# ModelTC/llmc

Hardware: AMD Instinct MI355X
Metric: layers/sec (GPTQ W4A16, Llama-3-8B Linear shapes, 128x2048 calib) (higher is better)
Workload: dtype bf16

## Files before the change

llmc_amd/_ffi.py:

```python
import ctypes as C
import os

import torch

_HERE = os.path.dirname(os.path.abspath(__file__))
LIB_PATH = os.path.join(_HERE, 'csrc', 'libllmc_hip.so')

F16, BF16, F32 = 0, 1, 2
F64 = 3
OUT_FAKE, OUT_I32, OUT_I8, OUT_U8 = 0, 1, 2, 3
SCALAR_QPARAM = 16
LINEAR_YBLOCKED = 4
FRACTIONAL_ZP = 32

_DT = {torch.float16: F16, torch.bfloat16: BF16, torch.float32: F32}

_i64, _i32, _f32, _f64, _vp, _sz = C.c_int64, C.c_int, C.c_float, C.c_double, C.c_void_p, C.c_size_t

SIGNATURES = {
    'llmc_hip_abi_version': (_i32, []),
    'llmc_hip_build_id': (C.c_char_p, []),
    'llmc_hip_last_error': (_i32, [C.c_char_p, _sz]),
    'llmc_hip_set_helper_streams': (_i32, [_i32]),
    'llmc_hip_set_cu_reserve': (_i32, [_i32]),
    'llmc_hip_set_option': (_i32, [C.c_char_p, _i32]),
    'llmc_hip_get_option': (_i32, [C.c_char_p]),
    'llmc_hip_option_name': (_i32, [_i32, C.c_char_p, _sz]),
    'llmc_minmax_qparams_ws_bytes': (_sz, [_i64, _i64]),
    'llmc_minmax_qparams': (_i32, [_vp, _i32, _i64, _i64, _i32, _i32, _f32, _f32, _vp, _vp, _vp, _vp]),
    'llmc_minmax_samples_max': (_i32, []),
    'llmc_minmax_samples_ws_bytes': (_sz, [_vp, _i32]),
    'llmc_minmax_samples': (_i32, [_vp, _vp, _i32, _i32, _vp, _vp, _vp, _vp]),
    'llmc_histc_ws_bytes': (_sz, [_i32]),
    'llmc_histc': (_i32, [_vp, _i32, _i64, _i32, _f32, _f32, _vp, _vp, _vp]),
    'llmc_mse_qparams': (_i32, [_vp, _i32, _i64, _i64, _i32, _i32, _f32, _f32, _i32, _i32, _f32, _vp, _vp, _vp, _vp, _vp]),
    'llmc_mse_qparams_panel': (_i32, [_vp, _i64, _i64, _i64, _i64, _i64, _i32, _i32, _f32, _f32, _i32, _i32, _f32, _vp,
                                      _vp, _i64, _i64, _vp]),
    'llmc_hqq_ws_bytes': (_sz, [_i64, _i64, _i32, _i64, _i32]),
    'llmc_hqq_optimize': (_i32, [_vp, _i32, _i64, _i64, _i64, _i32, _i64, _i32, _i32, _f32, _f32, _vp, _vp, _f32, _f32,
                                 _i32, _i32, _vp, _vp, _vp, _vp, _vp, _vp]),
    'llmc_quant_static': (_i32, [_vp, _i32, _i64, _i64, _vp, _i32, _vp, _i32, _f32, _f32, _i32, _vp, _vp]),
    'llmc_quant_dynamic_ws_bytes': (_sz, [_i64, _i64]),
    'llmc_quant_dynamic': (_i32, [_vp, _i32, _i64, _i64, _i32, _i32, _f32, _f32, _i32, _vp, _vp, _vp, _vp, _vp]),
    'llmc_pack_lsb': (_i32, [_vp, _i32, _i64, _i64, _i32, _vp, _vp]),
    'llmc_hessian_accum_ws_bytes': (_sz, [_i64, _i64, _i64]),
    'llmc_hessian_accum': (_i32, [_vp, _vp, _i32, _i64, _i64, _i64, _f64, _f64, _vp, _vp]),
    'llmc_hessian_accum_partials': (_i32, [_vp, _i32, _i64, _i64, _i64, _vp, _vp]),
    'llmc_hessian_accum_reduce': (_i32, [_vp, _i64, _i64, _i64, _f64, _f64, _vp, _vp]),
    'llmc_hessian_max_samples': (_i32, []),
    'llmc_hessian_accum_ptrs_ws_bytes': (_sz, [_vp, _i32, _i64, _i64]),
    'llmc_hessian_accum_ptrs': (_i32, [_vp, _vp, _vp, _i32, _i32, _i64, _i64, _f64, _f64, _vp, _vp]),
    'llmc_hessian_accum_ptrs_partials': (_i32, [_vp, _vp, _i32, _i32, _i64, _i64, _vp, _vp]),
    'llmc_hessian_accum_ptrs_reduce': (_i32, [_vp, _vp, _i32, _i64, _i64, _f64, _f64, _vp, _vp]),
    'llmc_hessian_accum_barrier_timeouts': (_i32, [_vp, _vp, _i32, _i64, _i64, _vp, _vp]),
    'llmc_hessian_max_problems': (_i32, []),
    'llmc_hessian_accum_multi_ws_bytes': (_sz, [_vp, _i32]),
    'llmc_hessian_accum_multi_partials': (_i32, [_vp, _i32, _i32, _vp, _vp]),
    'llmc_hessian_accum_multi_reduce': (_i32, [_vp, _i32, _vp, _vp]),
    'llmc_hessian_accum_multi_barrier_timeouts': (_i32, [_vp, _i32, _vp, _vp, _vp]),
    'llmc_gather_cols': (_i32, [_vp, _i64, _i64, _vp, _vp, _vp]),
    'llmc_hessian_prep_ws_bytes': (_sz, [_i64]),
    'llmc_hessian_prep': (_i32, [_vp, _vp, _i32, _i64, _i64, _vp, _f32, _vp, _vp, _vp, _vp]),
    'llmc_chol_inv_upper_ws_bytes': (_sz, [_i64]),
    'llmc_chol_inv_upper': (_i32, [_vp, _i64, _vp, _vp, _vp]),
    'llmc_hessian_prep_rev': (_i32, [_vp, _vp, _i32, _i64, _i64, _vp, _f32, _vp, _vp, _vp, _vp]),
    'llmc_chol_inv_upper_rev': (_i32, [_vp, _vp, _i64, _vp, _vp, _vp]),
    'llmc_gptq_quantize_ws_bytes': (_sz, [_i64, _i64]),
    'llmc_gptq_quantize': (_i32, [_vp, _vp, _i64, _i64, _i32, _f32, _f32, _i64, _i32, _vp, _vp, _vp, _vp, _vp,
                                  _i32, _vp, _vp]),
    'llmc_gptq_quantize_cols': (_i32, [_vp, _vp, _i64, _i64, _i64, _i32, _f32, _f32, _i64, _i32, _vp, _vp, _vp, _vp, _vp,
                                       _i32, _vp, _vp]),
    'llmc_gptq_quantize_fp8_cols': (_i32, [_vp, _vp, _i64, _i64, _i64, _i32, _i64, _i32, _vp, _vp, _vp, _vp, _i32, _vp, _vp]),
    'llmc_gptq_quantize_mse_ws_bytes': (_sz, [_i64, _i64]),
    'llmc_gptq_quantize_mse': (_i32, [_vp, _vp, _i64, _i64, _i64, _i32, _f32, _f32, _i64, _i32, _i32, _i32, _f32, _vp, _vp,
                                      _vp, _vp, _i32, _vp, _vp]),
    'llmc_spqr_quantize_ws_bytes': (_sz, [_i64, _i64]),
    'llmc_spqr_quantize': (_i32, [_vp, _vp, _i64, _i64, _f32, _f32, _i64, _f32, _i32, _f32, _f32, _f32, _f32, _vp, _vp,
                                  _vp, _vp, _vp, _i32, _vp, _vp]),
    'llmc_awq_act_mean_ws_bytes': (_sz, [_i64, _i64]),
    'llmc_awq_act_mean': (_i32, [_vp, _i32, _i64, _i64, _vp, _vp, _vp]),
    'llmc_awq_weight_mean_ws_bytes': (_sz, [_i64, _i64]),
    'llmc_awq_weight_mean': (_i32, [_vp, _i32, _i64, _i64, _i64, _vp, _vp, _vp]),
    'llmc_awq_scales': (_i32, [_vp, _vp, _i32, _i64, _f64, _i32, _vp, _vp]),
    'llmc_awq_scale_fakequant': (_i32, [_vp, _vp, _i32, _i64, _i64, _i64, _i32, _f32, _f32, _vp, _vp]),
    'llmc_div_cols': (_i32, [_vp, _vp, _i32, _i64, _i64, _vp, _vp]),
    'llmc_div_cols_kt': (_i32, [_vp, _vp, _i32, _i64, _i64, _vp, _vp]),
    'llmc_mul_cols': (_i32, [_vp, _vp, _i32, _i64, _i64, _vp]),
    'llmc_clamp_groups': (_i32, [_vp, _i32, _i64, _i64, _i64, _vp, _vp, _vp]),
    'llmc_linear_eval_ws_bytes': (_sz, [_i64, _i64, _i64]),
    'llmc_linear_eval': (_i32, [_vp, _vp, _i32, _i64, _i64, _i64, _i32, _vp, _vp, _vp, _vp, _vp]),
    'llmc_linear_eval_yblocked_bytes': (_sz, [_i64, _i64]),
    'llmc_ktile_pack': (_i32, [_vp, _i32, _i64, _i64, _vp, _vp]),
    'llmc_linear_eval_kt': (_i32, [_vp, _vp, _i32, _i64, _i64, _i64, _i32, _vp, _vp, _vp, _vp, _vp]),
    'llmc_awq_clip_search_ws_bytes': (_sz, [_i64, _i64, _i64, _i64]),
    'llmc_awq_clip_search': (_i32, [_vp, _vp, _i32, _i64, _i64, _i64, _i64, _i32, _i32, _i32, _i32, _f32, _f32,
                                    _vp, _vp, _vp, _vp]),
    'llmc_awq_clip_errs': (_i32, [_vp, _vp, _i32, _i64, _i64, _i64, _i64, _i32, _i32, _i32, _i32, _f32, _f32, _vp, _vp]),
    'llmc_awq_clip_errs_cand': (_i32, [_vp, _vp, _vp, _vp, _i32, _i64, _i64, _i64, _i64, _i64, _i32, _vp, _vp]),
    'llmc_fp8_quant_ws_bytes': (_sz, [_i64, _i64]),
    'llmc_fp8_quant': (_i32, [_vp, _i32, _i64, _i64, _i32, _vp, _vp, _i32, _i32, _vp, _vp]),
    'llmc_fpx_quant_ws_bytes': (_sz, [_i64, _i64]),
    'llmc_fpx_quant': (_i32, [_vp, _i32, _i64, _i64, _vp, _i64, _i32, _vp, _vp, _i32, _i32, _vp, _vp]),
    'llmc_fp4_pack': (_i32, [_vp, _i64, _i64, _vp, _vp]),
    'llmc_fpx_dequant': (_i32, [_vp, _i32, _i32, _vp, _i32, _i64, _i64, _vp, _i32, _vp]),
    'llmc_fp8_block_quant': (_i32, [_vp, _i32, _i64, _i64, _i32, _f32, _i32, _vp, _vp, _vp]),
    'llmc_fp8_block_dequant': (_i32, [_vp, _vp, _i64, _i64, _i32, _i32, _vp, _vp]),
    'llmc_fp8_act_quant': (_i32, [_vp, _i32, _i64, _i32, _vp, _vp, _vp]),
    'llmc_fp8_block_gemm': (_i32, [_vp, _vp, _vp, _vp, _i64, _i64, _i64, _i32, _vp, _vp, _vp]),
    'llmc_pack_awq_gemm': (_i32, [_vp, _i32, _vp, _i32, _vp, _i64, _i64, _i64, _vp, _vp, _vp, _vp]),
    'llmc_col_stats_ws_bytes': (_sz, [_i64, _i64]),
    'llmc_col_stats': (_i32, [_vp, _i32, _i64, _i64, _i32, _vp, _vp, _vp, _vp]),
    'llmc_smooth_scales': (_i32, [_vp, _vp, _i32, _i64, _f64, _f64, _vp, _vp]),
    'llmc_osplus_scale': (_i32, [_vp, _vp, _vp, _i64, _i32, _i64, _vp, _vp]),
    'llmc_osplus_act_step_tier': (_i32, [_i32, _i64]),
    'llmc_osplus_act_step': (_i32, [_vp, _vp, _i32, _i64, _i64, _i32, _i32, _f32, _f32, _i32, _vp, _vp]),
    'llmc_hadamard': (_i32, [_vp, _vp, _i32, _i64, _i64, _i64, _vp, _i32, _f64, _vp]),
    'llmc_test_sgemm': (_i32, [_vp, _vp, _vp, _i64, _i64, _i64, _i32, _i32, _i32, _i32, _i32, _i32, _i32, _i32,
                               _i32, _i32, _vp]),
    'llmc_test_sgemm_phased': (_i32, [_vp, _vp, _vp, _i64, _i64, _i64, _i32, _i32, _i32, _i32, _i32, _vp]),
    'llmc_test_gemm3': (_i32, [_vp, _vp, _vp, _i64, _i64, _i64, _i32, _i32, _i32, _i32, _i32, _i32, _i32, _i32, _vp]),
    'llmc_test_gemm3_planes': (_i32, [_vp, _vp, _vp, _i64, _i64, _i64, _i32, _i32, _i32, _i32, _i32, _vp, _vp]),
    'llmc_test_gemm3s_stamps': (_i32, [_vp]),
    'llmc_test_gptq_rider_plan': (_i32, [_i64, _i64, _i64, _i64, _i32, _vp, _i32]),
    'llmc_test_gptq_pipe_plan': (_i32, [_i64, _i64, _i64, _i64, _i32, _vp, _i32]),
    'llmc_test_chol_plan': (_i32, [_i64, _i32, _i32, _vp, _i32]),
    'llmc_test_gemm_route': (_i32, [_vp, _vp]),
}



class HessianProblem(C.Structure):
    _fields_ = [('H', _vp), ('dstate', _vp), ('X_list_host', _vp), ('T_list_host', _vp), ('n', _i32), ('K', _i64),
                ('ldx', _i64), ('n_before', _f64), ('n_after', _f64)]


_lib = None


class LlmcHipError(RuntimeError):
    pass


def lib():
    global _lib
    if _lib is None:
        if not os.path.exists(LIB_PATH):
            raise LlmcHipError(
                f'{LIB_PATH} not found: the HIP extension is required (run `python -m llmc_amd.build`). '
                'llmc_amd has no CPU fallback.')
        handle = C.CDLL(LIB_PATH)
        for name, (res, args) in SIGNATURES.items():
            fn = getattr(handle, name)
            fn.restype = res
            fn.argtypes = args
        ver = handle.llmc_hip_abi_version()
        if ver != 1:
            raise LlmcHipError(f'libllmc_hip.so ABI version {ver} != 1')
        if not os.environ.get('LLMC_SKIP_BUILD_ID_CHECK'):
            from . import build as _build
            have, want = handle.llmc_hip_build_id().decode(), _build.source_digest()
            if have != want:
                raise LlmcHipError(f'{LIB_PATH} is stale: built from sources {have}, csrc/ is {want} '
                                   '(run `python -m llmc_amd.build`; LLMC_SKIP_BUILD_ID_CHECK=1 skips this check)')
        _lib = handle
        _apply_startup_options()
    return _lib


HOST_OPTIONS = {
    'awq_kt': 1,
    'awq_y_bytes': (1 << 32) - (1 << 20),
    'k3_fused_prep': 1,
}

_HOST_DEFAULTS = dict(HOST_OPTIONS)


def reset_options():
    HOST_OPTIONS.update(_HOST_DEFAULTS)
    if _lib is not None:
        for k in library_options():
            _lib.llmc_hip_set_option(k.encode(), 0)


def set_option(key, value):
    if key in HOST_OPTIONS:
        prev, HOST_OPTIONS[key] = HOST_OPTIONS[key], int(value)
        return prev
    prev = lib().llmc_hip_set_option(key.encode(), int(value))
    if prev < 0:
        raise ValueError(f'unknown option {key!r} (library keys: {library_options()}; host keys: {sorted(HOST_OPTIONS)})')
    return prev


def get_option(key):
    if key in HOST_OPTIONS:
        return HOST_OPTIONS[key]
    v = lib().llmc_hip_get_option(key.encode())
    if v < 0:
        raise ValueError(f'unknown option {key!r}')
    return v


def library_options():
    out, buf, i = [], C.create_string_buffer(64), 0
    while lib().llmc_hip_option_name(i, buf, 64) > 0:
        out.append(buf.value.decode())
        i += 1
    return out


class option:

    def __init__(self, **kv):
        self.kv = kv

    def __enter__(self):
        self.prev = {k: set_option(k, v) for k, v in self.kv.items()}
        return self

    def __exit__(self, *exc):
        for k, v in self.prev.items():
            set_option(k, v)
        return False


def _apply_startup_options():
    spec = os.environ.get('LLMC_OPTIONS', '')
    for item in filter(None, (x.strip() for x in spec.split(','))):
        k, _, v = item.partition('=')
        set_option(k.strip(), int(v or 1))


def last_error():
    buf = C.create_string_buffer(512)
    lib().llmc_hip_last_error(buf, 512)
    return buf.value.decode(errors='replace')


def check(rc, what):
    if rc == 0:
        return
    msg = last_error()
    if rc == -22:
        raise ValueError(f'{what}: invalid argument: {msg}')
    if rc == -95:
        raise NotImplementedError(f'{what}: unsupported: {msg}')
    raise LlmcHipError(f'{what}: HIP error: {msg}')


def dt(t):
    try:
        return _DT[t.dtype if isinstance(t, torch.Tensor) else t]
    except KeyError:
        raise ValueError(f'unsupported dtype {t.dtype if isinstance(t, torch.Tensor) else t}')


def require_gpu(*tensors):
    cur = None
    for t in tensors:
        if t is None:
            continue
        if not t.is_cuda:
            raise LlmcHipError(
                'llmc_amd operators run on MI355X only (tensor is on '
                f'{t.device}); there is no CPU fallback. Use oracle/ for CPU checks in tests.')
        if cur is None:
            cur = torch.cuda.current_device()
        if t.device.index != cur:
            raise LlmcHipError(f'tensor lives on {t.device} but the current device is cuda:{cur}: wrap the call in '
                               '`with torch.cuda.device(tensor.device)` (hipSetDevice is the caller\'s job)')


def ptr(t):
    return 0 if t is None else t.data_ptr()


def stream():
    return torch.cuda.current_stream().cuda_stream


def workspace(nbytes, device):
    if nbytes <= 0:
        return None
    return torch.empty(int(nbytes), dtype=torch.uint8, device=device)


class helper_streams:

    def __init__(self, enable):
        self.enable = int(bool(enable))

    def __enter__(self):
        self.prev = lib().llmc_hip_set_helper_streams(self.enable)

    def __exit__(self, *exc):
        lib().llmc_hip_set_helper_streams(self.prev)
        return False


class cu_reserve:

    def __init__(self, n):
        self.n = int(n)

    def __enter__(self):
        self.prev = lib().llmc_hip_set_cu_reserve(self.n)

    def __exit__(self, *exc):
        lib().llmc_hip_set_cu_reserve(self.prev)
        return False
```

llmc_amd/csrc/abi.hip:

```cpp
#include <mutex>
#include <set>
#include <utility>
#include "common.h"

namespace llmc {
static thread_local char g_last_error[512] = "";
static thread_local int g_helper_streams = 1;
bool helper_streams_enabled() { return g_helper_streams != 0; }
static thread_local int g_cu_reserve = 0;
int cu_reserve() { return g_cu_reserve; }
static thread_local int g_opt[OPT_COUNT] = {};
int opt(int id) { return (id >= 0 && id < OPT_COUNT) ? g_opt[id] : 0; }
static const char* const g_opt_names[OPT_COUNT] = {
    "k3_fp32", "k3_no_gemm6", "k3_no_planes", "k3_split_far", "k4_split_far", "k4_err_rowmajor", "gptq_generic",
    "gemm3_nospec", "gemm3s_min_tiles", "no_shortk", "linear_nosplit", "fp8_exact_div", "side_cu_mask", "k1_batch_off", "k1_fp32_diag", "fp8_no_packed16", "gemm3s_no_dma", "sgemm_no_wide", "gemm3_no_wide", "no_riders"};

void set_last_error(const char* where, hipError_t e) {
    snprintf(g_last_error, sizeof(g_last_error), "%s: %s (%d)", where, hipGetErrorString(e), (int)e);
}
void set_last_error_msg(const char* msg) { snprintf(g_last_error, sizeof(g_last_error), "%s", msg); }

static std::mutex g_dev_mu;
static int g_cu_count[LLMC_MAX_DEVICES] = {};
static std::set<std::pair<int, const void*>> g_lds_attr_done;

int device_cu_count() {
    int dev = 0;
    if (hipGetDevice(&dev) != hipSuccess || dev < 0 || dev >= LLMC_MAX_DEVICES) return 256;
    std::lock_guard<std::mutex> lk(g_dev_mu);
    if (g_cu_count[dev] == 0) {
        int n = 0;
        if (hipDeviceGetAttribute(&n, hipDeviceAttributeMultiprocessorCount, dev) != hipSuccess || n <= 0) n = 256;
        g_cu_count[dev] = n;
    }
    return g_cu_count[dev];
}

int ensure_dynamic_lds(const void* fn, int bytes) {
    int dev = 0;
    LLMC_HIP_CHECK(hipGetDevice(&dev));
    std::lock_guard<std::mutex> lk(g_dev_mu);
    auto key = std::make_pair(dev, fn);
    if (g_lds_attr_done.count(key)) return LLMC_OK;
    LLMC_HIP_CHECK(hipFuncSetAttribute(fn, hipFuncAttributeMaxDynamicSharedMemorySize, bytes));
    g_lds_attr_done.insert(key);
    return LLMC_OK;
}
}

extern "C" int llmc_hip_set_helper_streams(int enable) {
    int prev = llmc::g_helper_streams;
    llmc::g_helper_streams = enable ? 1 : 0;
    return prev;
}

extern "C" int llmc_hip_set_option(const char* key, int value) {
    if (!key || value < 0) return LLMC_EINVAL;
    for (int i = 0; i < llmc::OPT_COUNT; ++i)
        if (strcmp(key, llmc::g_opt_names[i]) == 0) {
            const int prev = llmc::g_opt[i];
            llmc::g_opt[i] = value;
            return prev;
        }
    llmc::set_last_error_msg("llmc_hip_set_option: unknown key");
    return LLMC_EINVAL;
}

extern "C" int llmc_hip_get_option(const char* key) {
    if (!key) return LLMC_EINVAL;
    for (int i = 0; i < llmc::OPT_COUNT; ++i)
        if (strcmp(key, llmc::g_opt_names[i]) == 0) return llmc::g_opt[i];
    return LLMC_EINVAL;
}

extern "C" int llmc_hip_option_name(int index, char* buf_host, size_t n) {
    if (index < 0 || index >= llmc::OPT_COUNT || !buf_host || n == 0) return LLMC_EINVAL;
    strncpy(buf_host, llmc::g_opt_names[index], n - 1);
    buf_host[n - 1] = 0;
    return (int)strlen(buf_host);
}

extern "C" int llmc_hip_set_cu_reserve(int n_cus) {
    int prev = llmc::g_cu_reserve;
    llmc::g_cu_reserve = n_cus < 0 ? 0 : n_cus;
    return prev;
}

extern "C" int llmc_hip_abi_version(void) { return LLMC_HIP_ABI_VERSION; }

#ifndef LLMC_BUILD_ID
#define LLMC_BUILD_ID "unknown"
#endif
extern "C" const char* llmc_hip_build_id(void) { return LLMC_BUILD_ID; }

extern "C" int llmc_hip_last_error(char* buf_host, size_t n) {
    if (!buf_host || n == 0) return (int)strlen(llmc::g_last_error);
    strncpy(buf_host, llmc::g_last_error, n - 1);
    buf_host[n - 1] = 0;
    return (int)strlen(buf_host);
}
```

llmc_amd/csrc/common.h:

```cpp
#pragma once
#include <hip/hip_runtime.h>
#include <stdint.h>
#include <string.h>
#include <stdio.h>
#include <stdlib.h>

#include "../../include/llmc_hip.h"

namespace llmc {

void set_last_error(const char* where, hipError_t e);
void set_last_error_msg(const char* msg);

#define LLMC_HIP_CHECK(expr)                                   \
    do {                                                       \
        hipError_t _e = (expr);                                \
        if (_e != hipSuccess) {                                \
            ::llmc::set_last_error(#expr, _e);                 \
            return LLMC_EIO;                                   \
        }                                                      \
    } while (0)

#define LLMC_LAUNCH_CHECK()                                    \
    do {                                                       \
        hipError_t _e = hipGetLastError();                     \
        if (_e != hipSuccess) {                                \
            ::llmc::set_last_error("kernel launch", _e);       \
            return LLMC_EIO;                                   \
        }                                                      \
    } while (0)

#define LLMC_REQUIRE(cond, msg)                                \
    do {                                                       \
        if (!(cond)) {                                         \
            ::llmc::set_last_error_msg(msg);                   \
            return LLMC_EINVAL;                                \
        }                                                      \
    } while (0)

static constexpr int LLMC_MAX_DEVICES = 64;
int device_cu_count();
int ensure_dynamic_lds(const void* fn, int bytes);
int cu_reserve();
bool helper_streams_enabled();

enum Opt : int {
    OPT_K3_FP32 = 0,
    OPT_K3_NO_GEMM6,
    OPT_K3_NO_PLANES,
    OPT_K3_SPLIT_FAR,
    OPT_K4_SPLIT_FAR,
    OPT_K4_ERR_ROWMAJOR,
    OPT_GPTQ_GENERIC,
    OPT_GEMM3_NOSPEC,
    OPT_GEMM3S_MIN_TILES,
    OPT_NO_SHORTK,
    OPT_LINEAR_NOSPLIT,
    OPT_FP8_EXACT_DIV,
    OPT_SIDE_CU_MASK,
    OPT_K1_BATCH_OFF,
    OPT_K1_FP32_DIAG,
    OPT_FP8_NO_PACKED16,
    OPT_GEMM3S_NO_DMA,
    OPT_SGEMM_NO_WIDE,
    OPT_GEMM3_NO_WIDE,
    OPT_NO_RIDERS,
    OPT_COUNT
};
int opt(int id);
#ifdef LLMC_LAB
static inline const char* lab_env(const char* k) { return getenv(k); }
#endif

static inline int dtype_size(int dt) { return dt == LLMC_F32 ? 4 : 2; }
static inline bool dtype_ok(int dt) { return dt == LLMC_F16 || dt == LLMC_BF16 || dt == LLMC_F32; }

struct f16_t { uint16_t u; };
struct bf16_t { uint16_t u; };

template <typename T> struct dt_of;
template <> struct dt_of<f16_t> { static constexpr int value = LLMC_F16; };
template <> struct dt_of<bf16_t> { static constexpr int value = LLMC_BF16; };
template <> struct dt_of<float> { static constexpr int value = LLMC_F32; };

#define DISPATCH_DT(dt, ...)                                              \
    switch (dt) {                                                         \
        case LLMC_F16: { using T = ::llmc::f16_t; __VA_ARGS__; break; }   \
        case LLMC_BF16: { using T = ::llmc::bf16_t; __VA_ARGS__; break; } \
        default: { using T = float; __VA_ARGS__; break; }                 \
    }

__device__ __forceinline__ float f16_bits_to_f32(uint16_t u) {
    _Float16 h;
    __builtin_memcpy(&h, &u, 2);
    return (float)h;
}
__device__ __forceinline__ uint16_t f32_to_f16_bits(float v) {
    asm volatile("" : "+v"(v));
    _Float16 h = (_Float16)v;
    uint16_t u;
    __builtin_memcpy(&u, &h, 2);
    return u;
}
__device__ __forceinline__ float bf16_bits_to_f32(uint16_t u) {
    return __uint_as_float(((uint32_t)u) << 16);
}
__device__ __forceinline__ uint16_t f32_to_bf16_bits(float v) {
    const __bf16 h = (__bf16)v;
    uint16_t u;
    __builtin_memcpy(&u, &h, 2);
    return u;
}

__device__ __forceinline__ float opaque_f32(float v) {
    asm volatile("" : "+v"(v));
    return v;
}

__device__ __forceinline__ float rnd(float v, int dt) {
    if (dt == LLMC_F16) return f16_bits_to_f32(f32_to_f16_bits(v));
    if (dt == LLMC_BF16) return bf16_bits_to_f32(f32_to_bf16_bits(v));
    return v;
}
template <int DT> __device__ __forceinline__ float rndc(float v) {
    if constexpr (DT == LLMC_F16) return f16_bits_to_f32(f32_to_f16_bits(v));
    else if constexpr (DT == LLMC_BF16) return bf16_bits_to_f32(f32_to_bf16_bits(v));
    else return v;
}

__device__ __forceinline__ float load_as_f32(const void* p, int64_t i, int dt) {
    if (dt == LLMC_F16) return f16_bits_to_f32(((const uint16_t*)p)[i]);
    if (dt == LLMC_BF16) return bf16_bits_to_f32(((const uint16_t*)p)[i]);
    return ((const float*)p)[i];
}
__device__ __forceinline__ void store_from_f32(void* p, int64_t i, int dt, float v) {
    if (dt == LLMC_F16) ((uint16_t*)p)[i] = f32_to_f16_bits(v);
    else if (dt == LLMC_BF16) ((uint16_t*)p)[i] = f32_to_bf16_bits(v);
    else ((float*)p)[i] = v;
}

template <typename T> __device__ __forceinline__ float to_f32(T v);
template <> __device__ __forceinline__ float to_f32<f16_t>(f16_t v) { return f16_bits_to_f32(v.u); }
template <> __device__ __forceinline__ float to_f32<bf16_t>(bf16_t v) { return bf16_bits_to_f32(v.u); }
template <> __device__ __forceinline__ float to_f32<float>(float v) { return v; }

template <typename T> __device__ __forceinline__ T from_f32(float v);
template <> __device__ __forceinline__ f16_t from_f32<f16_t>(float v) { return f16_t{f32_to_f16_bits(v)}; }
template <> __device__ __forceinline__ bf16_t from_f32<bf16_t>(float v) { return bf16_t{f32_to_bf16_bits(v)}; }
template <> __device__ __forceinline__ float from_f32<float>(float v) { return v; }

__host__ __device__ __forceinline__ int promote(int a, int b) {
    if (a == b) return a;
    return LLMC_F32;
}

template <typename T> struct vec16 {
    static constexpr int N = 16 / sizeof(T);
    T v[N];
};

__device__ __forceinline__ float wave_max(float v, int width) {
    for (int o = width >> 1; o > 0; o >>= 1) v = fmaxf(v, __shfl_xor(v, o, 64));
    return v;
}
__device__ __forceinline__ float wave_min(float v, int width) {
    for (int o = width >> 1; o > 0; o >>= 1) v = fminf(v, __shfl_xor(v, o, 64));
    return v;
}
__device__ __forceinline__ float wave_sum(float v, int width) {
    for (int o = width >> 1; o > 0; o >>= 1) v += __shfl_xor(v, o, 64);
    return v;
}

static inline int64_t ceil_div64(int64_t a, int64_t b) { return (a + b - 1) / b; }
static inline int capped_grid(int64_t items, int64_t per_block, int64_t cap) {
    const int64_t b = ceil_div64(items, per_block);
    return (int)(b < 1 ? 1 : (b > cap ? cap : b));
}
static inline int pow2_ceil(int64_t x) {
    int p = 1;
    while (p < x) p <<= 1;
    return p;
}

}
```

llmc_amd/csrc/gptq_loop.hip:

```cpp
#include "gptq_block_kernels.h"
#include "pipe_lanes.h"

using namespace llmc;

static constexpr int GRP = 4;
static constexpr int GW = BS * GRP;

extern "C" size_t llmc_gptq_quantize_ws_bytes(int64_t R, int64_t K) {
    if (R <= 0 || K <= 0) return 0;
    return 3 * (size_t)((R + 3) & ~(int64_t)3) * GW * sizeof(float);
}

extern "C" int llmc_gptq_quantize(float* W, const float* Hinv, int64_t R, int64_t K, int sym, float qmin,
                                  float qmax, int64_t group_size, int static_groups, const int32_t* col_group,
                                  float* scales, float* zeros, float* Wout, float* losses, int blocksize,
                                  void* ws, llmc_stream_t stream) {
    return llmc_gptq_quantize_cols(W, Hinv, R, K, K, sym, qmin, qmax, group_size, static_groups, col_group, scales,
                                   zeros, Wout, losses, blocksize, ws, stream);
}

struct MseSearch { int round_zp, nsteps, grid; float norm; };

struct Piece { int64_t c0, c1; int k0, k1; Lane lane; };
static constexpr int CARRIERS = GRP;
static_assert(CARRIERS % RIDER_PASSES == 0 && GRP % RIDER_PASSES == 0, "a group's carrying launches and phases divide into the passes");

static int far_pieces(int64_t gend, int64_t K, bool merged, int rider_cols, Piece* p) {
    const int64_t gend2 = gend + GW < K ? gend + GW : K, gend3 = gend2 + GW < K ? gend2 + GW : K;
    if (!merged) {
        p[0] = Piece{gend, gend2, 0, GW, CHAIN}, p[1] = Piece{gend2, gend3, 0, GW, BULK}, p[2] = Piece{gend3, K, 0, GW, BULK};
        return 1 + (gend2 < K) + (gend3 < K);
    }
    const int64_t rw = (int64_t)rider_cols * 128, rspan = (CARRIERS / RIDER_PASSES) * rw;
    const int64_t p0 = (rider_cols > 0 && gend2 < K) ? (gend2 > K - rspan ? gend2 : K - rspan) : K;
    p[0] = Piece{gend, p0, 0, GW, CHAIN};
    int n = 1;
    const int kd = GW / RIDER_PASSES;
    for (int pass = 0; pass < RIDER_PASSES; ++pass)
        for (int64_t c = p0; c < K; c += rw) p[n++] = Piece{c, c + rw < K ? c + rw : K, pass * kd, (pass + 1) * kd, RIDE};
    return n;
}

struct ColCall {
    float* W; const float* U; float* Wout; float* losses; float* scales; float* zeros; const int32_t* col_group;
    int64_t R, K, NQ;
    bool ekm; int64_t Rp, err_ld; float* ErrBuf[3];
    int ng, gsz, static_mode, sym; float qmin, qmax;
    const MseSearch* mse;
    int kind;

    float* err(int group, int64_t k) const { return ErrBuf[group % 3] + (ekm ? k * Rp : k); }
    int64_t group_end(int64_t g0) const { return g0 + GW < NQ ? g0 + GW : NQ; }
    int64_t near_end(int64_t g0) const { return group_end(g0) == NQ ? K : group_end(g0); }
    int count(int64_t i1) const { return (int)(NQ - i1 < BS ? NQ - i1 : BS); }

    GptqBlockArgs block(int64_t i1) const {
        GptqBlockArgs a;
        a.W = W; a.U = U; a.Wout = Wout; a.losses = losses;
        a.Err = err((int)(i1 / GW), i1 % GW); a.err_ld = (int)err_ld; a.err_kmajor = ekm ? 1 : 0;
        a.scales = scales; a.zeros = zeros; a.col_group = mse ? nullptr : col_group; a.col_gsz = mse ? gsz : 1 << 30;
        a.R = R; a.K = (int)K; a.i1 = (int)i1; a.count = count(i1); a.ng = ng; a.gsz = static_mode ? BS : gsz;
        a.static_mode = static_mode; a.sym = sym; a.qmin = qmin; a.qmax = qmax;
        return a;
    }
    SgemmArgs product(const float* A, int64_t row0, int kd, int64_t c0, int64_t c1, int phase_len) const {
        SgemmArgs g{};
        g.A = A; g.lda = err_ld; g.B = U + row0 * K + c0; g.ldb = K; g.C = W + c0; g.ldc = K;
        g.M = g.M_last = (int)R; g.N = g.N_last = (int)(c1 - c0); g.Kd = g.Kd_last = kd;
        g.epilogue = SG_SUB; g.batch = 1; g.phase_len = phase_len;
        return g;
    }
    SgemmArgs near(int64_t i1) const {
        const int64_t g0 = i1 - i1 % GW, c0 = (i1 + count(i1)) & ~(int64_t)3;
        return product(err((int)(i1 / GW), i1 % GW), i1, count(i1), c0, near_end(g0), 0);
    }
    SgemmArgs far(int group, int64_t c0, int64_t c1, int k0, int k1) const {
        return product(err(group, k0), (int64_t)group * GW + k0, k1 - k0, c0, c1, BS);
    }
    RiderArgs riders(int group, const Piece& q, int nchain) const {
        RiderArgs ra{};
        wide::wide_operands<2>(far(group, q.c0, q.c1, q.k0, q.k1), ra.w);
        ra.nchain = nchain; ra.per = (nchain % 8 == 0 && ra.w.tm % 8 == 0) ? ra.w.tm / 8 : 0;
        return ra;
    }
};

enum { PLAN_BLOCK = 0, PLAN_NEAR = 1, PLAN_NEAR_FAR = 2, PLAN_FAR = 3, PLAN_FLUSH = 4, PLAN_W = 12 };
static const int32_t PLAN_BLANK[PLAN_W] = {0, 0, 0, 0, -1, -1, -1, 0, 0, -1, 0, 0};

struct Sink {
    const ColCall& o; const Lanes& ln; PlanRec* rec;
    void add(int lane, int kind, int group, int64_t w0, int64_t w1, int err_rd, int err_wr, int rgroup, int64_t r0, int64_t r1, int rerr,
             int k0, int k1) const {
        const int32_t v[PLAN_W] = {kind, group, (int32_t)w0, (int32_t)w1, err_rd, err_wr, rgroup, (int32_t)r0, (int32_t)r1, rerr, k0, k1};
        rec->row(v, lane);
    }
    int err_index(const float* pe) const { return (int)((size_t)(pe - o.ErrBuf[0]) / ((size_t)o.Rp * GW)); }
    void k_range(int group, const float* B, int64_t c0, int kd, int* k0, int* k1) const {
        *k0 = (int)((B - o.U - c0) / o.K - (int64_t)group * GW);
        *k1 = *k0 + kd;
        if (kd == GW) *k0 = *k1 = 0;
    }
    int product(int kind, int group, const SgemmArgs& g, hipStream_t st) const {
        if (!rec) return sgemm_launch(g, o.ekm, false, st);
        const int64_t c0 = g.C - o.W;
        int k0 = 0, k1 = 0;
        if (kind != PLAN_NEAR) k_range(group, g.B, c0, g.Kd, &k0, &k1);
        add(ln.lane_of(st), kind, group, c0, c0 + g.N, err_index(g.A), -1, -1, 0, 0, -1, k0, k1);
        return LLMC_OK;
    }
    int in_block(int group, const GptqBlockArgs& a, int variant, int nt, int grid, const RiderArgs* ra, int rgroup) const {
        const hipStream_t st = ln.s[CHAIN];
        if (rec) {
            int64_t r0 = 0, r1 = 0;
            int rerr = -1, k0 = 0, k1 = 0;
            if (ra) {
                r0 = ra->w.C - o.W, r1 = r0 + (int64_t)ra->w.tn * 128, rerr = err_index(ra->w.A);
                k_range(rgroup, ra->w.B, r0, ra->w.nst * wide::W_K, &k0, &k1);
            }
            add(CHAIN, PLAN_BLOCK, group, a.i1, a.i1 + a.count, -1, err_index(a.Err), rgroup, r0, r1, rerr, k0, k1);
            return LLMC_OK;
        }
        return o.kind == QK_E4M3 ? gptq_launch_in_block_e4m3(a, variant, nt, grid, ra, st)
             : o.kind == QK_E5M2 ? gptq_launch_in_block_e5m2(a, variant, nt, grid, ra, st)
                                 : launch_in_block<QK_INT>(a, variant, nt, grid, ra, st);
    }
};

static int rider_quota(const ColCall& o, bool merged, int nt, int grid) {
    if (!merged || opt(OPT_NO_RIDERS) || !o.ekm || nt != GBT || o.R % 128 || o.K % 128 || o.NQ <= GW || o.K <= 2 * (int64_t)GW) return 0;
    const int free_cus = device_cu_count() - grid;
    if (sgemm_route(o.far(0, 2 * GW, o.K, 0, GW), true, false).wide_form != 2 || free_cus <= 0 || 2 * grid < device_cu_count()) return 0;
    return (int)(free_cus / (o.R / 128));
}

static int gptq_cols_impl(float* W, const float* Hinv, int64_t R, int64_t K, int64_t n_quant, int sym, float qmin,
                          float qmax, int64_t group_size, int static_groups, const int32_t* col_group, float* scales,
                          float* zeros, float* Wout, float* losses, int blocksize, void* ws, llmc_stream_t stream,
                          const MseSearch* mse, PlanRec* rec = nullptr, int kind = QK_INT) {
    LLMC_REQUIRE(W && Hinv && Wout && scales && ws && R > 0 && K > 0, "gptq_quantize: null/empty argument");
    LLMC_REQUIRE(n_quant > 0 && n_quant <= K, "gptq_quantize: n_quant must be in (0, K]");
    LLMC_REQUIRE(blocksize == BS, "gptq_quantize: blocksize must be 128");
    LLMC_REQUIRE(K % 4 == 0 && K < (1 << 30), "gptq_quantize: K must be a multiple of 4");
    LLMC_REQUIRE(sym || zeros, "gptq_quantize: zeros required for asymmetric");
    const bool per_channel = group_size <= 0;
    const int static_mode = static_groups || per_channel || mse != nullptr;
    const int gsz = (int)group_size;
    if (!static_mode || mse) {
        if (!(gsz == 16 || gsz == 32 || gsz == 64 || gsz == 128)) {
            set_last_error_msg("gptq_quantize: dynamic group qparams need group_size in {16,32,64,128}");
            return LLMC_ENOTSUP;
        }
    } else if (!per_channel) {
        LLMC_REQUIRE(col_group != nullptr, "gptq_quantize: col_group required with static groups");
    }
    const bool ekm = !opt(OPT_K4_ERR_ROWMAJOR);
    const int64_t Rp = (R + 3) & ~(int64_t)3;
    const ColCall o{W, Hinv, Wout, losses, scales, zeros, per_channel ? nullptr : col_group, R, K, n_quant,
                    ekm, Rp, ekm ? Rp : GW, {(float*)ws, (float*)ws + (size_t)Rp * GW, (float*)ws + 2 * (size_t)Rp * GW},
                    per_channel ? 1 : (int)ceil_div64(K, group_size), gsz, static_mode, sym, qmin, qmax, mse, kind};
    Lanes ln((hipStream_t)stream, rec);
    const Sink sink{o, ln, rec};
    const bool merged = !ln.piped() && !opt(OPT_K4_SPLIT_FAR);
    const int nt = R >= 16384 ? 1024 : GBT;
    const int grid = (int)ceil_div64(R, nt / 16);
    const int rider_cols = rider_quota(o, merged, nt, grid);
    const bool force_generic = opt(OPT_GPTQ_GENERIC) != 0;
    Piece pc[1 + CARRIERS];
    int np = 0, next = 0, fg = 0;
    auto flush = [&]() -> int {
        for (; next < np; ++next)
            LLMC_TRY(sink.product(PLAN_FLUSH, fg, o.far(fg, pc[next].c0, pc[next].c1, pc[next].k0, pc[next].k1), ln.s[CHAIN]));
        return LLMC_OK;
    };
    Ev reached_next{};
    Ev err_read[3] = {};
    Ev bulk_tail{};
    LLMC_TRY(ln.fork());
    int g = 0;
    for (int64_t g0 = 0; g0 < o.NQ; g0 += GW, ++g) {
        const int64_t gend = o.group_end(g0), near_end = o.near_end(g0);
        if (near_end > gend) {
            LLMC_TRY(flush());
            LLMC_TRY(ln.wait(CHAIN, bulk_tail));
        }
        LLMC_TRY(ln.wait(CHAIN, err_read[g % 3]));
        for (int64_t i1 = g0; i1 < gend; i1 += BS) {
            const GptqBlockArgs a = o.block(i1);
            const int variant = (a.count != BS || force_generic) ? 0 : static_mode ? 1 : gsz == BS ? BS : 0;
            if (mse && !rec) {
                LLMC_TRY(llmc_mse_qparams_panel(W, R, K, i1, a.count, gsz, sym, mse->round_zp, qmin, qmax, mse->nsteps, mse->grid,
                                                mse->norm, scales, zeros, o.ng, i1 / gsz, (llmc_stream_t)ln.s[CHAIN]));
            }
            const bool ride = next < np;
            const RiderArgs ra = ride ? o.riders(fg, pc[next++], grid) : RiderArgs{};
            LLMC_TRY(sink.in_block(g, a, variant, nt, grid, ride ? &ra : nullptr, ride ? fg : -1));
            if (i1 + a.count < near_end) LLMC_TRY(sink.product(PLAN_NEAR, g, o.near(i1), ln.s[CHAIN]));
        }
        if (near_end == K) continue;
        LLMC_TRY(ln.wait(CHAIN, reached_next));
        reached_next = Ev{};
        LLMC_TRY(flush());
        np = far_pieces(gend, K, merged, rider_cols, pc);
        fg = g;
        int nbulk = 0;
        for (next = 0; next < np && pc[next].lane != RIDE; ++next) {
            const Piece& p = pc[next];
            if (p.lane == BULK && nbulk == 0) LLMC_TRY(ln.order(CHAIN, BULK));
            const int kind = (p.lane == CHAIN && !merged) ? PLAN_NEAR_FAR : PLAN_FAR;
            LLMC_TRY(sink.product(kind, g, o.far(g, p.c0, p.c1, p.k0, p.k1), ln.s[p.lane]));
            if (p.lane == BULK && nbulk++ == 0) LLMC_TRY(ln.record(BULK, &reached_next));
        }
        if (nbulk) {
            LLMC_TRY(ln.record(BULK, &err_read[g % 3]));
            bulk_tail = err_read[g % 3];
        }
    }
    LLMC_TRY(flush());
    return ln.join();
}

extern "C" int llmc_gptq_quantize_cols(float* W, const float* Hinv, int64_t R, int64_t K, int64_t n_quant, int sym,
                                       float qmin, float qmax, int64_t group_size, int static_groups,
                                       const int32_t* col_group, float* scales, float* zeros, float* Wout,
                                       float* losses, int blocksize, void* ws, llmc_stream_t stream) {
    return gptq_cols_impl(W, Hinv, R, K, n_quant, sym, qmin, qmax, group_size, static_groups, col_group, scales, zeros,
                          Wout, losses, blocksize, ws, stream, nullptr);
}

extern "C" int llmc_gptq_quantize_fp8_cols(float* W, const float* Hinv, int64_t R, int64_t K, int64_t n_quant, int fmt,
                                           int64_t group_size, int static_groups, const int32_t* col_group, float* scales,
                                           float* Wout, float* losses, int blocksize, void* ws, llmc_stream_t stream) {
    if (fmt != 0 && fmt != 1) {
        set_last_error_msg("gptq_quantize_fp8_cols: fmt must be 0 (e4m3) or 1 (e5m2)");
        return LLMC_ENOTSUP;
    }
    const float qmax = fmt ? 57344.0f : 448.0f;
    return gptq_cols_impl(W, Hinv, R, K, n_quant, 1, -qmax, qmax, group_size, static_groups, col_group, scales, nullptr, Wout,
                          losses, blocksize, ws, stream, nullptr, nullptr, fmt ? QK_E5M2 : QK_E4M3);
}

extern "C" size_t llmc_gptq_quantize_mse_ws_bytes(int64_t R, int64_t K) { return llmc_gptq_quantize_ws_bytes(R, K); }

extern "C" int llmc_gptq_quantize_mse(float* W, const float* Hinv, int64_t R, int64_t K, int64_t n_quant, int sym,
                                      float qmin, float qmax, int64_t group_size, int round_zp, int nsteps, int grid,
                                      float norm, float* scales, float* zeros, float* Wout, float* losses,
                                      int blocksize, void* ws, llmc_stream_t stream) {
    LLMC_REQUIRE(nsteps >= 1 && grid >= 1, "gptq_quantize_mse: nsteps and grid must be positive");
    if (!(group_size == 16 || group_size == 32 || group_size == 64 || group_size == 128)) {
        set_last_error_msg("gptq_quantize_mse: the searched group qparams need group_size in {16,32,64,128}");
        return LLMC_ENOTSUP;
    }
    const MseSearch m{round_zp, nsteps, grid, norm};
    return gptq_cols_impl(W, Hinv, R, K, n_quant, sym, qmin, qmax, group_size, 0, nullptr, scales, zeros, Wout, losses,
                          blocksize, ws, stream, &m);
}

static int gptq_plan(int64_t R, int64_t K, int64_t n_quant, int64_t group_size, int static_groups, int32_t* out, int cap, bool lanes) {
    LLMC_REQUIRE(out && cap >= 0, "gptq plan: null output");
    PlanRec rec{out, cap, 0, PLAN_W, lanes, PLAN_BLANK};
    float* const base = (float*)(uintptr_t)((uint64_t)1 << 40);
    const size_t span = (size_t)1 << 36;
    int32_t* cg = (int32_t*)(base + 6 * span);
    int rc = gptq_cols_impl(base, base + span, R, K, n_quant, 0, 0.0f, 15.0f, group_size, static_groups, cg, base + 2 * span,
                            base + 3 * span, base + 4 * span, nullptr, BS, base + 5 * span, nullptr, nullptr, &rec);
    return rc ? rc : rec.n;
}
extern "C" int llmc_test_gptq_rider_plan(int64_t R, int64_t K, int64_t n_quant, int64_t group_size, int static_groups, int32_t* out, int cap) {
    return gptq_plan(R, K, n_quant, group_size, static_groups, out, cap, false);
}
extern "C" int llmc_test_gptq_pipe_plan(int64_t R, int64_t K, int64_t n_quant, int64_t group_size, int static_groups, int32_t* out, int cap) {
    return gptq_plan(R, K, n_quant, group_size, static_groups, out, cap, true);
}
```

Measured before the change: 81.59.

## Add row-parallel GPTQ in-block kernel for large-R layers

Adds a new in-block GPTQ kernel that assigns each weight row to a quad of four lanes. Each lane keeps 32 columns in registers and uses DPP quad broadcasts to propagate the error across the 128-column block, with the upper-triangular U slice staged in LDS. The kernel is used by default when R is at least 16384, the block is full-width, the mode is integer static or group-128, and no riders are attached to that block. A slower exact path is kept as a fallback for non-finite or non-positive values. The aim is to cut per-block sequential cost for tall matrices such as MLP up/gate projections, at the price of losing rider overlap on those blocks and adding high register pressure.

```diff
diff --git a/llmc_amd/_ffi.py b/llmc_amd/_ffi.py
--- a/llmc_amd/_ffi.py
+++ b/llmc_amd/_ffi.py
@@ -125,6 +125,7 @@
     'llmc_test_gptq_pipe_plan': (_i32, [_i64, _i64, _i64, _i64, _i32, _vp, _i32]),
     'llmc_test_chol_plan': (_i32, [_i64, _i32, _i32, _vp, _i32]),
     'llmc_test_gemm_route': (_i32, [_vp, _vp]),
+    'llmc_test_inblock_rows_stats': (_i32, [_vp, _i32]),
 }
 
 
diff --git a/llmc_amd/csrc/abi.hip b/llmc_amd/csrc/abi.hip
--- a/llmc_amd/csrc/abi.hip
+++ b/llmc_amd/csrc/abi.hip
@@ -13,7 +13,7 @@
 int opt(int id) { return (id >= 0 && id < OPT_COUNT) ? g_opt[id] : 0; }
 static const char* const g_opt_names[OPT_COUNT] = {
     "k3_fp32", "k3_no_gemm6", "k3_no_planes", "k3_split_far", "k4_split_far", "k4_err_rowmajor", "gptq_generic",
-    "gemm3_nospec", "gemm3s_min_tiles", "no_shortk", "linear_nosplit", "fp8_exact_div", "side_cu_mask", "k1_batch_off", "k1_fp32_diag", "fp8_no_packed16", "gemm3s_no_dma", "sgemm_no_wide", "gemm3_no_wide", "no_riders"};
+    "gemm3_nospec", "gemm3s_min_tiles", "no_shortk", "linear_nosplit", "fp8_exact_div", "side_cu_mask", "k1_batch_off", "k1_fp32_diag", "fp8_no_packed16", "gemm3s_no_dma", "sgemm_no_wide", "gemm3_no_wide", "no_riders", "inblock_rows"};
 
 void set_last_error(const char* where, hipError_t e) {
     snprintf(g_last_error, sizeof(g_last_error), "%s: %s (%d)", where, hipGetErrorString(e), (int)e);
diff --git a/llmc_amd/csrc/common.h b/llmc_amd/csrc/common.h
--- a/llmc_amd/csrc/common.h
+++ b/llmc_amd/csrc/common.h
@@ -65,6 +65,7 @@
     OPT_SGEMM_NO_WIDE,
     OPT_GEMM3_NO_WIDE,
     OPT_NO_RIDERS,
+    OPT_INBLOCK_ROWS,
     OPT_COUNT
 };
 int opt(int id);
diff --git a/llmc_amd/csrc/gptq_block_rows.h b/llmc_amd/csrc/gptq_block_rows.h
--- /dev/null
+++ b/llmc_amd/csrc/gptq_block_rows.h
@@ -0,0 +1,14 @@
+#pragma once
+#include "gptq_block_kernels.h"
+
+namespace llmc {
+
+static constexpr int64_t ROWS_MIN_R = 16384;
+
+static inline bool in_block_rows_eligible(const GptqBlockArgs& a, int variant, int kind) {
+    return kind == QK_INT && a.count == BS && (variant == 1 || variant == BS);
+}
+
+int gptq_launch_in_block_rows(const GptqBlockArgs& a, int variant, hipStream_t st);
+
+}
diff --git a/llmc_amd/csrc/gptq_block_rows.hip b/llmc_amd/csrc/gptq_block_rows.hip
--- /dev/null
+++ b/llmc_amd/csrc/gptq_block_rows.hip
@@ -0,0 +1,239 @@
+#include <atomic>
+#include "gptq_block_rows.h"
+#include "../../include/llmc_hip_test.h"
+
+namespace llmc {
+
+static constexpr int RL = 4;
+static constexpr int RC = BS / RL;
+static constexpr int RNT = 256;
+
+__device__ unsigned int g_rows_fallback_waves;
+static std::atomic<long long> g_rows_launches{0};
+
+template <int Q> __device__ __forceinline__ float quad_bcast(float v) {
+    return __int_as_float(__builtin_amdgcn_update_dpp(0, __float_as_int(v), Q * 0x55, 0xf, 0xf, false));
+}
+
+template <int I, bool FAST, bool STATIC>
+__device__ __forceinline__ void rows_step(float (&w)[RC], float (&df)[RC], const float (&sc)[RC], const float (&zr)[RC],
+                                          const float* __restrict__ us, const float2* __restrict__ dtab, int q, float s_cur,
+                                          float z_cur, float y_cur, float qmin, float qmax) {
+    constexpr int M0 = I >> 4, QI = (I >> 2) & 3, JI = M0 * 4 + (I & 3);
+    typedef float v2f __attribute__((ext_vector_type(2)));
+    float4 u[8];
+#pragma unroll
+    for (int m = M0; m < 8; ++m) u[m] = *reinterpret_cast<const float4*>(us + I * BS + m * 4);
+    const float2 dd = dtab[I];
+    float s = s_cur, z = z_cur, y = y_cur;
+    if (STATIC) {
+        s = quad_bcast<QI>(sc[JI]);
+        z = quad_bcast<QI>(zr[JI]);
+        if (FAST) y = rcp_refined(s);
+    }
+    const float wi = quad_bcast<QI>(w[JI]);
+    float diff, err;
+    if (FAST) {
+        float t = div_tail(wi, s, y);
+        t = rintf(t);
+        t = t + z;
+        const float qc = fminf(fmaxf(t, qmin), qmax);
+        const float qv = (qc - z) * s;
+        diff = wi - qv;
+        err = div_tail(diff, dd.x, dd.y);
+    } else {
+        const float qc = quant_code(wi, s, z, LLMC_F32, LLMC_F32, qmin, qmax);
+        const float qv = dequant_code(qc, s, z, LLMC_F32);
+        diff = wi - qv;
+        err = diff / dd.x;
+    }
+    df[JI] = (q == QI) ? diff : df[JI];
+    asm volatile("" : "+v"(df[JI]));
+#pragma unroll
+    for (int m = M0; m < 8; ++m) {
+        const v2f ua = {u[m].x, u[m].y}, ub = {u[m].z, u[m].w};
+        v2f wa = {w[4 * m], w[4 * m + 1]}, wb = {w[4 * m + 2], w[4 * m + 3]};
+        const v2f ta = ua * err;
+        const v2f tb = ub * err;
+        wa = wa - ta;
+        wb = wb - tb;
+        w[4 * m] = wa.x;
+        w[4 * m + 1] = wa.y;
+        w[4 * m + 2] = wb.x;
+        w[4 * m + 3] = wb.y;
+    }
+    __builtin_amdgcn_sched_barrier(0);
+}
+
+template <bool FAST, bool STATIC>
+__device__ __forceinline__ bool rows_block(const GptqBlockArgs& a, const float* __restrict__ Us, const float2* __restrict__ dtab,
+                                           int q, int64_t row, bool active) {
+    const int64_t rr = active ? row : a.R - 1;
+    float w[RC], df[RC], sc[RC], zr[RC];
+    bool bad = false;
+    const float* wp = a.W + rr * a.K + a.i1 + 4 * q;
+#pragma unroll
+    for (int m = 0; m < 8; ++m) {
+        const float4 v = *reinterpret_cast<const float4*>(wp + 16 * m);
+        w[4 * m] = v.x;
+        w[4 * m + 1] = v.y;
+        w[4 * m + 2] = v.z;
+        w[4 * m + 3] = v.w;
+    }
+#pragma unroll
+    for (int j = 0; j < RC; ++j) {
+        df[j] = 0.0f;
+        sc[j] = 1.0f;
+        zr[j] = 0.0f;
+        if (STATIC) {
+            const int c = 16 * (j >> 2) + 4 * q + (j & 3);
+            const int g = a.col_group ? a.col_group[a.i1 + c] : (a.i1 + c) / a.col_gsz;
+            sc[j] = a.scales[rr * a.ng + g];
+            zr[j] = a.zeros ? a.zeros[rr * a.ng + g] : 0.0f;
+            if (FAST) bad |= !plain_pos(sc[j]);
+        }
+    }
+    float s_cur = 1.0f, z_cur = 0.0f, y_cur = 1.0f;
+    if (!STATIC) {
+        float mn = INFINITY, mx = -INFINITY;
+#pragma unroll
+        for (int j = 0; j < RC; ++j) {
+            mn = fminf(mn, w[j]);
+            mx = fmaxf(mx, w[j]);
+        }
+        mn = wave_min(mn, RL);
+        mx = wave_max(mx, RL);
+        const QParams qp = qparams_from_minmax(mn, mx, LLMC_F32, a.sym, 1, a.qmin, a.qmax);
+        s_cur = qp.s;
+        z_cur = qp.z;
+        if (FAST) {
+            y_cur = rcp_refined(s_cur);
+            bad |= !plain_pos(s_cur);
+        }
+    }
+    const float* us = Us + q * RC;
+#define LLMC_RSTEP(I) rows_step<I, FAST, STATIC>(w, df, sc, zr, us, dtab, q, s_cur, z_cur, y_cur, a.qmin, a.qmax);
+#define LLMC_RSTEP16(B)                                                                                                   \
+    LLMC_RSTEP(B + 0) LLMC_RSTEP(B + 1) LLMC_RSTEP(B + 2) LLMC_RSTEP(B + 3) LLMC_RSTEP(B + 4) LLMC_RSTEP(B + 5)           \
+    LLMC_RSTEP(B + 6) LLMC_RSTEP(B + 7) LLMC_RSTEP(B + 8) LLMC_RSTEP(B + 9) LLMC_RSTEP(B + 10) LLMC_RSTEP(B + 11)         \
+    LLMC_RSTEP(B + 12) LLMC_RSTEP(B + 13) LLMC_RSTEP(B + 14) LLMC_RSTEP(B + 15)
+    LLMC_RSTEP16(0) LLMC_RSTEP16(16) LLMC_RSTEP16(32) LLMC_RSTEP16(48) LLMC_RSTEP16(64) LLMC_RSTEP16(80) LLMC_RSTEP16(96)
+    LLMC_RSTEP16(112)
+#undef LLMC_RSTEP16
+#undef LLMC_RSTEP
+    if (FAST) {
+#pragma unroll
+        for (int j = 0; j < RC; ++j) bad |= !plain_num(w[j]) | !plain_num(df[j]);
+        if (__any(bad)) return false;
+    }
+    if (!active) return true;
+    float* wo = a.Wout + row * a.K + a.i1 + 4 * q;
+    float* lo = a.losses ? a.losses + row * a.K + a.i1 + 4 * q : nullptr;
+#pragma unroll
+    for (int m = 0; m < 8; ++m) {
+        *reinterpret_cast<float4*>(wo + 16 * m) = make_float4(w[4 * m], w[4 * m + 1], w[4 * m + 2], w[4 * m + 3]);
+        const int c = 16 * m + 4 * q;
+        float er[4], ls[4];
+#pragma unroll
+        for (int t = 0; t < 4; ++t) {
+            const float2 dd = dtab[c + t];
+            const float diff = df[4 * m + t];
+            er[t] = FAST ? div_tail(diff, dd.x, dd.y) : diff / dd.x;
+            ls[t] = (diff * diff) / (2.0f * (dd.x * dd.x));
+        }
+        if (lo) *reinterpret_cast<float4*>(lo + 16 * m) = make_float4(ls[0], ls[1], ls[2], ls[3]);
+        if (a.err_kmajor) {
+#pragma unroll
+            for (int t = 0; t < 4; ++t) a.Err[(int64_t)(c + t) * a.err_ld + row] = er[t];
+        } else {
+            *reinterpret_cast<float4*>(a.Err + row * a.err_ld + c) = make_float4(er[0], er[1], er[2], er[3]);
+        }
+    }
+    if (!STATIC && q == 0) {
+        const int g = a.i1 / BS;
+        a.scales[row * a.ng + g] = s_cur;
+        if (a.zeros) a.zeros[row * a.ng + g] = z_cur;
+    }
+    return true;
+}
+
+template <int VARIANT>
+__global__ __launch_bounds__(RNT) void k_gptq_block_rows(GptqBlockArgs a) {
+    __shared__ __attribute__((aligned(16))) float Us[BS * BS];
+    __shared__ float2 dtab[BS];
+    __shared__ int d_not_plain;
+    const int tid = threadIdx.x;
+    if (tid == 0) d_not_plain = 0;
+    __syncthreads();
+    {
+        constexpr int NV = BS * BS / 4 / RNT / 2;
+#pragma unroll
+        for (int h = 0; h < 2; ++h) {
+            float4 v[NV];
+#pragma unroll
+            for (int j = 0; j < NV; ++j) {
+                const int idx = tid + RNT * (j + NV * h);
+                const int i = idx >> 5, c4 = (idx & 31) * 4;
+                v[j] = *reinterpret_cast<const float4*>(a.U + (int64_t)(a.i1 + i) * a.K + a.i1 + c4);
+            }
+#pragma unroll
+            for (int j = 0; j < NV; ++j) {
+                const int idx = tid + RNT * (j + NV * h);
+                const int i = idx >> 5, c4 = (idx & 31) * 4;
+                const float vv[4] = {v[j].x, v[j].y, v[j].z, v[j].w};
+                float o[4];
+#pragma unroll
+                for (int t = 0; t < 4; ++t) {
+                    const int c = c4 + t;
+                    if (c == i) {
+                        dtab[i] = make_float2(vv[t], rcp_refined(vv[t]));
+                        if (!plain_pos(vv[t])) d_not_plain = 1;
+                    }
+                    o[t] = c > i ? vv[t] : 0.0f;
+                }
+                *reinterpret_cast<float4*>(&Us[i * BS + ((c4 >> 2) & 3) * RC + (c4 >> 4) * 4]) = make_float4(o[0], o[1], o[2], o[3]);
+            }
+        }
+    }
+    __syncthreads();
+
+    const int lane = tid & 63;
+    const int q = lane & (RL - 1);
+    const int64_t row0 = ((int64_t)blockIdx.x * (RNT / 64) + (tid >> 6)) * (64 / RL);
+    if (row0 >= a.R) return;
+    const int64_t row = row0 + (lane >> 2);
+    const bool active = row < a.R;
+    constexpr bool STATIC = VARIANT == 1;
+    if (!d_not_plain) {
+        if (rows_block<true, STATIC>(a, Us, dtab, q, row, active)) return;
+    }
+    if (lane == 0) atomicAdd(&g_rows_fallback_waves, 1u);
+    rows_block<false, STATIC>(a, Us, dtab, q, row, active);
+}
+
+int gptq_launch_in_block_rows(const GptqBlockArgs& a, int variant, hipStream_t st) {
+    const int grid = (int)ceil_div64(a.R, RNT / RL);
+    if (variant == 1) hipLaunchKernelGGL((k_gptq_block_rows<1>), dim3(grid), dim3(RNT), 0, st, a);
+    else hipLaunchKernelGGL((k_gptq_block_rows<BS>), dim3(grid), dim3(RNT), 0, st, a);
+    LLMC_LAUNCH_CHECK();
+    g_rows_launches.fetch_add(1, std::memory_order_relaxed);
+    return LLMC_OK;
+}
+
+}
+
+extern "C" int llmc_test_inblock_rows_stats(int64_t* out_host, int reset) {
+    using namespace llmc;
+    LLMC_REQUIRE(out_host != nullptr, "inblock_rows_stats: null output");
+    unsigned int fb = 0;
+    LLMC_HIP_CHECK(hipDeviceSynchronize());
+    LLMC_HIP_CHECK(hipMemcpyFromSymbol(&fb, HIP_SYMBOL(g_rows_fallback_waves), sizeof(fb)));
+    out_host[0] = (int64_t)g_rows_launches.load(std::memory_order_relaxed);
+    out_host[1] = (int64_t)fb;
+    if (reset) {
+        const unsigned int zero = 0;
+        LLMC_HIP_CHECK(hipMemcpyToSymbol(HIP_SYMBOL(g_rows_fallback_waves), &zero, sizeof(zero)));
+        g_rows_launches.store(0, std::memory_order_relaxed);
+    }
+    return LLMC_OK;
+}
diff --git a/llmc_amd/csrc/gptq_loop.hip b/llmc_amd/csrc/gptq_loop.hip
--- a/llmc_amd/csrc/gptq_loop.hip
+++ b/llmc_amd/csrc/gptq_loop.hip
@@ -1,4 +1,5 @@
 #include "gptq_block_kernels.h"
+#include "gptq_block_rows.h"
 #include "pipe_lanes.h"
 
 using namespace llmc;
@@ -109,7 +110,7 @@
         add(ln.lane_of(st), kind, group, c0, c0 + g.N, err_index(g.A), -1, -1, 0, 0, -1, k0, k1);
         return LLMC_OK;
     }
-    int in_block(int group, const GptqBlockArgs& a, int variant, int nt, int grid, const RiderArgs* ra, int rgroup) const {
+    int in_block(int group, const GptqBlockArgs& a, int variant, int nt, int grid, const RiderArgs* ra, int rgroup, bool rows) const {
         const hipStream_t st = ln.s[CHAIN];
         if (rec) {
             int64_t r0 = 0, r1 = 0;
@@ -121,6 +122,7 @@
             add(CHAIN, PLAN_BLOCK, group, a.i1, a.i1 + a.count, -1, err_index(a.Err), rgroup, r0, r1, rerr, k0, k1);
             return LLMC_OK;
         }
+        if (rows) return gptq_launch_in_block_rows(a, variant, st);
         return o.kind == QK_E4M3 ? gptq_launch_in_block_e4m3(a, variant, nt, grid, ra, st)
              : o.kind == QK_E5M2 ? gptq_launch_in_block_e5m2(a, variant, nt, grid, ra, st)
                                  : launch_in_block<QK_INT>(a, variant, nt, grid, ra, st);
@@ -166,6 +168,8 @@
     const int grid = (int)ceil_div64(R, nt / 16);
     const int rider_cols = rider_quota(o, merged, nt, grid);
     const bool force_generic = opt(OPT_GPTQ_GENERIC) != 0;
+    const int rows_opt = opt(OPT_INBLOCK_ROWS);
+    const bool rows_on = rows_opt == 1 || (rows_opt == 0 && R >= ROWS_MIN_R);
     Piece pc[1 + CARRIERS];
     int np = 0, next = 0, fg = 0;
     auto flush = [&]() -> int {
@@ -194,7 +198,8 @@
             }
             const bool ride = next < np;
             const RiderArgs ra = ride ? o.riders(fg, pc[next++], grid) : RiderArgs{};
-            LLMC_TRY(sink.in_block(g, a, variant, nt, grid, ride ? &ra : nullptr, ride ? fg : -1));
+            const bool rows = rows_on && !ride && in_block_rows_eligible(a, variant, kind);
+            LLMC_TRY(sink.in_block(g, a, variant, nt, grid, ride ? &ra : nullptr, ride ? fg : -1, rows));
             if (i1 + a.count < near_end) LLMC_TRY(sink.product(PLAN_NEAR, g, o.near(i1), ln.s[CHAIN]));
         }
         if (near_end == K) continue;
```

Result: no change. 81.94, median of 6 (+0.4%).
